# siliconsorcery/crdt

Hardware: AMD Instinct MI355X
Metric: merged records/sec (node) + % HBM roofline, 1B records x 1024 replicas (higher is better)
Workload: dtype int64

## Files before the change

crdt_amd/csrc/crdt_merge.hip:

```cpp
#include <dlfcn.h>
#include <hip/hip_runtime.h>
#include <rccl/rccl.h>

#include <stdint.h>
#include <stdio.h>
#include <stdlib.h>
#include <string.h>

#include <unistd.h>

#include <algorithm>
#include <atomic>
#include <chrono>
#include <thread>
#include <new>
#include <vector>

#include "crdt_merge.h"

namespace {

constexpr int kShift = 16;
constexpr int64_t kMaxCounter = 0xFFFF;
constexpr int64_t kMaxDrift = 60000;
// ... 1752 lines not shown
    uint32_t form_off = 0;
    bool env_dynamic = false;
    bool hist_fuse = true;
    uint32_t l1_tile = 0;
    uint32_t plan_l1_tile = 28672;
    bool last_hist1_fused = false;
    bool frame_lt_only = false;
    const uint32_t* d_ptb = nullptr;
    uint64_t plan_ptiles = 0;
    DBuf<uint32_t> p_hist1;
    bool hist1_fused = false;
    bool hist1_routed = false;
    const uint32_t* hist1_key = nullptr;
    uint32_t hist1_shift = 0;
    bool last_packed = false;
    bool last_wire_pk = false;
    bool last_own_in_place = false;
    bool last_key8 = false;
    bool last_key16 = false;
    bool last_compact = false;
    bool last_hw = false;
    bool flags_sorted = true;
    int fback_chk = 6;
    bool last_flagged = false;
    int combine = 1;
    bool last_combined = false;
    uint32_t sparse_t = 2048;
    uint32_t hot_buckets = 256;
    uint32_t hot_share = 5;
    uint32_t hot_probe = kHotProbe;
    uint32_t hot_skip = 0;
    uint32_t hist1_hot = 0;
    bool last_hot_direct = false;
    DBuf<uint32_t> p_hist1h, p_toffh, p_dstarth;
    DBuf<uint64_t> p_l1begh;
    int route_l1 = 1;
    bool rl1_call_head = false;
    bool rl1_call_all = false;
    bool rl1_cmp = false;
    bool last_rl1_head = false;
    uint64_t last_rl1_head_in = 0, last_rl1_head_out = 0;
    uint32_t last_rl1_head_digits = 0;
    uint64_t sent_bytes = 0;
    uint32_t rl1_pieces = 2;
    uint32_t rl1_call_pieces = 2;
    uint32_t last_rl1_pieces = 0;
    bool last_route_l1 = false;
    bool route_tune = true;
    struct RouteTune {
        uint64_t shape = 0;
        uint32_t trial = 0;
        int best = -1;
        long long us[5] = {-1, -1, -1, -1, -1};
    } rt;
    int tune_mode = -1;
    bool tune_trial = false;
    DBuf<long long> d_tune;
    HBuf<long long> h_tune;
    DBuf<uint32_t> rl_rec;
    DBuf<uint16_t> rl_k16;
    uint64_t rl_cap = 0;
    Rl1Scratch rl_os[kRl1MaxPieces + 1];
    Rl1Scratch rl_hf;
    DBuf<uint32_t> rl_hrec;
    DBuf<uint16_t> rl_hk16;
    DBuf<unsigned long long> rl_hcnt;
// ... 630 lines not shown
                 crdt_result* out, uint8_t* dflags = nullptr,
                 EmitOut* emit = nullptr) {
    const uint32_t R = c->plan_R;
    const bool fl = dflags != nullptr;
    const bool em = emit != nullptr;
    if (!em) {
        if (!c->resolved)
            k_resolve<<<1, 64, 0, c->stream>>>(d_event, R, wall, c->canonical, c->d_Rj.p, c->d_Cj.p, c->d_misc);
        c->resolved = false;
        ev_record(c, kEvApply);
        c->windows.clear();
        c->apply_total = 1;
        if (c->timing) ev_record(c, ev_window(0, false));
    }
    const bool two = c->cap > (1ull << 20);
    const uint32_t shift1 = two ? 20u : (uint32_t)kSBits;
    const size_t ns_all = sg.j.size();
    PackFrame pf{};
    bool pk = false;
    if (cols.packed_in || (c->packed_resolve && c->frame_on)) {
        HIPCHK(hipMemcpyAsync(c->h_misc, c->d_misc, sizeof(Misc), hipMemcpyDeviceToHost, c->stream));
        SYNCHK(c, c->stream);
        pf = frame_of(c);
        pk = pf.ok;
        if (cols.packed_in && !pk) return CRDT_E_INVALID;
    }
    if ((fl || em) && (!pk || cols.packed_in)) return CRDT_E_INVALID;
    const bool ord = !em && (fl || (c->counts && pk && !cols.packed_in));
    c->last_ordered = ord;
    c->last_packed = pk;
    c->key_end_valid = true;
    c->last_hist1_fused = false;
    c->last_hot_direct = false;
    c->sorted_phases = false;
    const bool k8 = pk && two && pf.key4 && !(c->form_off & kFormNoKey8);
    const bool k16 = k8 && !(c->form_off & kFormNoKey16);
    bool cmp = false;
    if (k16 && (ord || !c->counts) && !em && !c->has_comm && !cols.packed_in && c->frame_on &&
        !(c->form_off & (kFormNoCompact | kFormNoHistW | kFormBigTile2 | kFormNoWholeLines | kFormNoVecLoads))) {
        const PackFrame cf = compact_frame(pf, (uint32_t)std::min<unsigned long long>(c->h_misc->fr_cmax, 0xFFFFull),
                                           c->plan_R);
        if (cf.cb) {
            pf = cf;
            cmp = true;
        }
    }
    c->last_compact = cmp;
    c->last_key8 = k8;
    c->last_key16 = k16;
    c->last_hw = pk && (!c->counts || ord) && c->hw_read < c->cap;
    const uint32_t win0 = pk ? pf.jwin : kWindow;
    const bool pt1 = fl && cmp && ns_all && sg.j[0] / win0 == sg.j[ns_all - 1] / win0 &&
                     !(c->form_off & (kFormNoPosT | kFormNoFbackPre | kFormFbackWide)) &&
                     !(c->xcd_map && (c->form_off & kFormFbackXcd));
    if (fl && !pt1) {
        uint64_t ncol = 0;
        for (size_t s = 0; s < ns_all; ++s) ncol = std::max<uint64_t>(ncol, sg.end[s]);
        HIPALLOC(c->f_pos1.ensure((ncol ? ncol : 1) + 8));
    }
    for (size_t sb = 0; sb < ns_all;) {
        const uint32_t win = pk ? pf.jwin : kWindow;
        const uint32_t jb = sg.j[sb] - sg.j[sb] % win;
        size_t se = sb;
        uint64_t nw = 0;
        while (se < ns_all && sg.j[se] < jb + win) { nw += sg.end[se] - sg.beg[se]; ++se; }
        const uint32_t nseg = (uint32_t)(se - sb);
// ... 55 lines not shown
            }
            for (hipEvent_t& e : c->place_ev)
                if (!e) HIPCHK(hipEventCreate(&e));
            c->place_timed = true;
        }
        HIPALLOC(c->p1_rec.ensure(rec_units)); HIPALLOC(c->p1_kj.ensure(kj1_units));
        u32x4* p1r = c->p1_rec.p;
        uint32_t* p1k = c->p1_kj.p;
        u32x4* p2r = nullptr;
        uint32_t* p2k = nullptr;
        const uint64_t* d_beg = c->p_plan.p;
        const uint64_t* d_end = c->p_plan.p + nseg;
        const uint32_t* d_sj = reinterpret_cast<const uint32_t*>(c->p_plan.p + 2 * (size_t)nseg);
        const uint32_t* d_tb1 = d_sj + nseg;
        HIPALLOC(c->p_tseg.ensure(ntm));
        k_seg_index<<<std::min<uint32_t>(grid_for(nt1, 256), 4096), 256, 0, c->stream>>>(d_tb1, nseg, nt1, c->p_tseg.p);
        const TileMap tm1{d_beg, d_end, d_tb1, c->p_tseg.p, d_sj, nseg, l1t};
        const ScanMap sm1z{reinterpret_cast<const uint32_t*>(c->p_plan.p + tail),
                          reinterpret_cast<const uint32_t*>(c->p_plan.p + tail + 1), c->p_plan.p + tail + 2, 1};
        if (two) HIPALLOC(c->p_l1beg.ensure(kDigits + 1));
        const bool h1 = c->hist1_fused && !c->hist1_routed && s0 == 0 && se == ns_all && !cols.packed_in &&
                        cols.key == c->hist1_key && c->hist1_shift == shift1 && nt1 == c->plan_ptiles &&
                        l1t == l1_plan_tile(c);
        const uint32_t* hist1 = h1 ? c->p_hist1.p : c->p_hist.p;
        const uint32_t hb = h1 ? c->hist1_hot : 0u;
        const uint64_t hot_n = hb && pk ? std::min<uint64_t>(c->h_misc->hot_n, nw) : 0;
        const bool hotp = hb && cmp && !ord && !em && two && !c->has_comm && hot_n * 100 >= (uint64_t)c->hot_share * nw;
        if (hb && !hotp) {
            k_hot_fold<<<std::min<uint32_t>(nt1, 1024u), 64, 0, c->stream>>>(c->p_hist1.p, c->p_hist1h.p, nt1);
            c->hist1_hot = 0;
            c->hot_skip = c->hot_probe;
        }
        c->last_hot_direct = hotp;
        if (hotp) {
            HIPALLOC(c->p_toffh.ensure((size_t)nt1 * kDigits));
            HIPALLOC(c->p_dstarth.ensure(kDigits + 1));
            HIPALLOC(c->p_l1begh.ensure(kDigits + 1));
            HIPALLOC(c->p2_rec.ensure(rec_units));
            k_hist_trim<<<256, 256, 0, c->stream>>>(c->p_hist1h.p, c->d_ptb, R, c->d_misc);
            k_scan_part<<<nc1, 256, 0, c->stream>>>(c->p_hist1h.p, sm1z, c->p_part.p);
            k_scan_seg<<<1, 256, 0, c->stream>>>(c->p_part.p, sm1z, c->p_choff.p, c->p_dstarth.p, c->p_l1begh.p);
            k_scan_tiles<<<nc1, 256, 0, c->stream>>>(c->p_hist1h.p, c->p_choff.p, sm1z, c->p_dstarth.p, c->p_toffh.p);
        }
        const ScanMap sm1 = hotp ? ScanMap{sm1z.tbase, sm1z.cbase, c->p_l1begh.p + kDigits, 1} : sm1z;
        if (h1)
            k_hist_trim<<<256, 256, 0, c->stream>>>(c->p_hist1.p, c->d_ptb, R, c->d_misc);
        else
            k_part_hist<true><<<nt1, kHThreads, 0, c->stream>>>(cols.key, tm1, jb, c->d_misc,
                                                                 c->cap, shift1, c->p_hist.p);
        c->last_hist1_fused = h1;
        k_scan_part<<<nc1, 256, 0, c->stream>>>(hist1, sm1, c->p_part.p);
        k_scan_seg<<<1, 256, 0, c->stream>>>(c->p_part.p, sm1, c->p_choff.p, c->p_dstart1.p,
                                             two ? c->p_l1beg.p : nullptr);
        k_scan_tiles<<<nc1, 256, 0, c->stream>>>(hist1, c->p_choff.p, sm1, c->p_dstart1.p, c->p_toff.p);
        const bool ph = c->timing && s0 == 0 && !em;
        if (ph) ev_record(c, ev_window(1, false));
        if (c->place_timed && s0 == 0) HIPCHK(hipEventRecord(c->place_ev[0], c->stream));
        const uint32_t xper1 = c->xcd_map ? (nt1 + kXcds - 1) / kXcds : 0;
        const bool rev1 = c->xcd_map && !(c->form_off & kFormNoReverse);
        if (pt1) HIPALLOC(c->f_pos1.ensure((size_t)nt1 * kPTile + 16));
        if (pt1)
            k_part_scatter1<true, false, true, kL1Items, true, true, true, true, true>
                <<<xcd_grid(nt1, c->xcd_map), kPThreads, 0, c->stream>>>(
                cols.key, cols.lt, cols.rank, cols.val, tm1, jb, c->d_misc, c->cap, shift1, c->p_toff.p, p1r,
                p1k, xper1, pf, rev1 ? hist1 : nullptr, c->f_pos1.p, hist1);
        else if (cmp && fl)
            k_part_scatter1<true, false, true, kL1Items, true, true, true, true>
                <<<xcd_grid(nt1, c->xcd_map), kPThreads, 0, c->stream>>>(
                cols.key, cols.lt, cols.rank, cols.val, tm1, jb, c->d_misc, c->cap, shift1, c->p_toff.p, p1r,
                p1k, xper1, pf, rev1 ? hist1 : nullptr, c->f_pos1.p, hist1);
        else if (hotp)
            k_part_scatter1<kL1Items><<<xcd_grid(nt1, c->xcd_map), kPThreads, 0, c->stream>>>(
                cols.key, cols.lt, cols.rank, cols.val, tm1, jb, c->d_misc, c->cap, shift1, c->p_toff.p, p1r,
                p1k, xper1, pf, rev1 ? hist1 : nullptr,
                HotL1{hb, c->p_toffh.p, rev1 ? c->p_hist1h.p : nullptr, c->p2_rec.p});
        else if (cmp)
            k_part_scatter1<true, false, true, kL1Items, true, true, false, true>
                <<<xcd_grid(nt1, c->xcd_map), kPThreads, 0, c->stream>>>(
                cols.key, cols.lt, cols.rank, cols.val, tm1, jb, c->d_misc, c->cap, shift1, c->p_toff.p, p1r,
                p1k, xper1, pf, rev1 ? hist1 : nullptr);
        else if (fl && k16)
            k_part_scatter1<true, false, true, kL1Items, true, true, true>
                <<<xcd_grid(nt1, c->xcd_map), kPThreads, 0, c->stream>>>(
                cols.key, cols.lt, cols.rank, cols.val, tm1, jb, c->d_misc, c->cap, shift1, c->p_toff.p, p1r,
                p1k, xper1, pf, rev1 ? hist1 : nullptr, c->f_pos1.p, hist1);
        else if (fl)
            k_part_scatter1<true, false, false, kL1Items, true, false, true>
                <<<xcd_grid(nt1, c->xcd_map), kPThreads, 0, c->stream>>>(
                cols.key, cols.lt, cols.rank, cols.val, tm1, jb, c->d_misc, c->cap, shift1, c->p_toff.p, p1r,
                p1k, xper1, pf, rev1 ? hist1 : nullptr, c->f_pos1.p, hist1);
        else if (cols.packed_in && k16)
            k_part_scatter1<true, true, true, kL1Items, true><<<xcd_grid(nt1, c->xcd_map), kPThreads, 0, c->stream>>>(
                cols.key, cols.lt, cols.rank, cols.val, tm1, jb, c->d_misc, c->cap, shift1, c->p_toff.p, p1r,
                p1k, xper1, pf, rev1 ? hist1 : nullptr);
        else if (cols.packed_in)
            k_part_scatter1<true, true, false, kL1Items, true><<<xcd_grid(nt1, c->xcd_map), kPThreads, 0, c->stream>>>(
                cols.key, cols.lt, cols.rank, cols.val, tm1, jb, c->d_misc, c->cap, shift1, c->p_toff.p, p1r,
                p1k, xper1, pf, rev1 ? hist1 : nullptr);
        else if (k16 && !(c->form_off & kFormNoVecLoads))
            k_part_scatter1<true, false, true, kL1Items, true><<<xcd_grid(nt1, c->xcd_map), kPThreads, 0, c->stream>>>(
                cols.key, cols.lt, cols.rank, cols.val, tm1, jb, c->d_misc, c->cap, shift1, c->p_toff.p, p1r,
                p1k, xper1, pf, rev1 ? hist1 : nullptr);
        else if (k16)
// ... 511 lines not shown
        case CRDT_E_NOMEM: return "device out of memory";
        case CRDT_E_KEY_RANGE: return "key id out of range";
        case CRDT_E_NO_DEVICE: return "no gfx950 device";
        case CRDT_E_COMM: return "communicator error";
        default: return "unknown status";
    }
}

int crdt_device_count(int* out) {
    if (!out) return CRDT_E_INVALID;
    int n = 0;
    if (hipGetDeviceCount(&n) != hipSuccess) n = 0;
    *out = n;
    return CRDT_OK;
}

static void read_env_knobs(crdt_ctx* c) {
    if (const char* e = getenv("CRDT_NO_FUSE")) c->no_fuse = atoi(e) != 0;
    if (const char* e = getenv("CRDT_XCD_MAP")) c->xcd_map = atoi(e) != 0;
    if (const char* e = getenv("CRDT_PACKED")) c->packed_resolve = atoi(e) != 0;
    if (const char* e = getenv("CRDT_FLAGS_SORTED")) c->flags_sorted = atoi(e) != 0;
    if (const char* e = getenv("CRDT_TABLE_MERGE")) c->table_merge = atoi(e) != 0;
    if (const char* e = getenv("CRDT_COMBINE")) c->combine = std::min(std::max(atoi(e), 0), 2);
    if (const char* e = getenv("CRDT_ROUTE_L1")) c->route_l1 = std::min(std::max(atoi(e), 0), 3);
    if (const char* e = getenv("CRDT_RL1_SPLIT")) {
        const int v = atoi(e);
        c->rl1_pieces = std::min<uint32_t>(v <= 0 ? 1u : v == 1 ? 2u : (uint32_t)v, kRl1MaxPieces);
    }
    if (const char* e = getenv("CRDT_ROUTE_TUNE")) c->route_tune = atoi(e) != 0;
    if (const char* e = getenv("CRDT_SPARSE_T")) c->sparse_t = (uint32_t)std::max(atoi(e), 0);
    if (const char* e = getenv("CRDT_HOT_BUCKETS")) c->hot_buckets = (uint32_t)std::min(std::max(atoi(e), 0), (int)kHotMax);
    if (const char* e = getenv("CRDT_HOT_PROBE")) c->hot_probe = (uint32_t)std::min(std::max(atoi(e), 0), 1 << 20);
    if (const char* e = getenv("CRDT_HOT_SHARE")) c->hot_share = (uint32_t)std::min(std::max(atoi(e), 0), 100);
    if (const char* e = getenv("CRDT_FBACK_CHK")) c->fback_chk = atoi(e) == 4 ? 4 : atoi(e) == 0 ? 0 : 6;
    if (const char* e = getenv("CRDT_HIST_FUSE")) c->hist_fuse = atoi(e) != 0;
    if (const char* e = getenv("CRDT_L1_TILE"))
        c->l1_tile = std::min<uint32_t>((uint32_t)std::max(atoi(e), 0) / 1024u * 1024u, (uint32_t)kPTile);
    if (const char* e = getenv("CRDT_SORTED_FORM")) c->form_off = (uint32_t)strtoul(e, nullptr, 10);
    if (const char* e = getenv("CRDT_APPLY_ITEMS")) {
        const int v = atoi(e);
        c->apply_items = (v == 1 || v == 2 || v == 4 || v == 8) ? v : 0;
    }
    c->fail_rank = -1;
    c->fail_at = 0;
    if (const char* e = getenv("CRDT_TEST_FAIL")) {
        int r = -1, at = 0;
        if (sscanf(e, "%d:%d", &r, &at) == 2) { c->fail_rank = r; c->fail_at = at; }
    }
    c->stall_rank = -1;
    c->stall_at = c->stall_ms = 0;
    c->stall_dev = false;
    if (const char* e = getenv("CRDT_TEST_STALL")) {
        int r = -1, at = 0, ms = 0;
        char d = 0;
        const int k = sscanf(e, "%d:%d:%d:%c", &r, &at, &ms, &d);
        if (k >= 3) { c->stall_rank = r; c->stall_at = at; c->stall_ms = ms; c->stall_dev = k == 4 && d == 'd'; }
    }
}

int crdt_create(int device, uint32_t local_rank, uint64_t capacity, crdt_ctx** out) {
    if (!out) return CRDT_E_INVALID;
    *out = nullptr;
    int n = 0;
    if (hipGetDeviceCount(&n) != hipSuccess || device < 0 || device >= n) return CRDT_E_NO_DEVICE;
    hipDeviceProp_t prop;
    if (hipGetDeviceProperties(&prop, device) != hipSuccess) return CRDT_E_NO_DEVICE;
// ... 1252 lines not shown
int crdt_set_merge_path(crdt_ctx* c, int path) {
    if (!c || path < CRDT_PATH_AUTO || path > CRDT_PATH_SORTED) return CRDT_E_INVALID;
    c->merge_path = path;
    return CRDT_OK;
}

int crdt_last_path(const crdt_ctx* c, int* path) {
    if (!c || !path) return CRDT_E_INVALID;
    *path = c->last_sorted ? CRDT_PATH_SORTED : CRDT_PATH_GATHER;
    return CRDT_OK;
}

int crdt_last_plan(const crdt_ctx* c, uint32_t* flags) {
    if (!c || !flags) return CRDT_E_INVALID;
    uint32_t f = 0;
    if (c->last_table_plan) {
        *flags = c->last_table_plan;
        return CRDT_OK;
    }
    if (c->last_sorted) {
        f |= CRDT_PLAN_SORTED;
        if (c->last_packed) f |= CRDT_PLAN_PACKED;
        if (c->cap > (1ull << 20)) f |= CRDT_PLAN_TWO_LEVEL;
        if (c->last_hist1_fused) f |= CRDT_PLAN_HIST_IN_SCAN;
        if (c->last_key8) f |= CRDT_PLAN_KEY8;
        if (c->last_key16) f |= CRDT_PLAN_KEY16;
        if (c->last_hw) f |= CRDT_PLAN_HIGH_WATER;
        if (c->last_flagged) f |= CRDT_PLAN_FLAGGED;
        if (c->last_ordered) f |= CRDT_PLAN_ORDERED;
        if (c->last_combined) f |= CRDT_PLAN_COMBINED;
        if (c->last_route_l1) f |= CRDT_PLAN_ROUTE_L1;
        if (c->last_compact) f |= CRDT_PLAN_COMPACT;
        if (c->last_hot_direct) f |= CRDT_PLAN_HOT_DIRECT;
    }
    if (c->last_wire_pk) f |= CRDT_PLAN_WIRE_PACKED;
    if (c->last_own_in_place) f |= CRDT_PLAN_OWN_IN_PLACE;
    if (c->tune_trial) f |= CRDT_PLAN_ROUTE_TUNED;
    if (c->last_route_l1) f |= (c->last_rl1_pieces & 7u) << CRDT_PLAN_RL1_PIECES_SHIFT;
    if (c->last_route_l1 && c->last_rl1_head) f |= CRDT_PLAN_RL1_HEAD;
    *flags = f;
    return CRDT_OK;
}

int crdt_place_info(const crdt_ctx* c, int32_t* n, int32_t* kept, int32_t* done, float* ms) {
    if (!c || !n || !kept || !done || !ms) return CRDT_E_INVALID;
    *n = c->place_k;
    *kept = c->place_best;
    *done = c->place_k > 1 ? c->place_trial + 1 : 0;
    for (int i = 0; i < crdt_ctx::kPlaceMax; ++i) ms[i] = i < c->place_k ? c->place_ms[i] : 0.f;
    return CRDT_OK;
}

int crdt_route_tune_info(const crdt_ctx* c, int32_t* best, int64_t* us) {
    if (!c || !best || !us) return CRDT_E_INVALID;
    *best = c->rt.best;
    for (int w = 0; w < 5; ++w) us[w] = c->rt.us[w];
    return CRDT_OK;
}

int crdt_set_timing(crdt_ctx* c, int enable) {
    if (!c) return CRDT_E_INVALID;
    c->timing = enable != 0;
    return CRDT_OK;
}

int crdt_get_timing(const crdt_ctx* c, crdt_timing* out) {
// ... 7 lines not shown
```

crdt_amd/csrc/sorted_path.inc:

```

constexpr int kSBits = 12;
constexpr uint32_t kSKeys = 1u << kSBits;
constexpr uint32_t kDigits = 256;
constexpr int kJShift = 20;
constexpr uint32_t kKeyLoMask = (1u << kJShift) - 1;
constexpr uint32_t kWindow = 1u << (32 - kJShift);
constexpr int kHThreads = 1024;
constexpr int kPThreads = 1024;
constexpr int kPWaves = kPThreads / 64;
constexpr int kPItems = 4;
constexpr int kPSub = kPThreads * kPItems;
constexpr int kPTile = 28672;
constexpr int kPTile2 = 8192;
constexpr int kPGroups = kPItems * kPWaves;
#ifndef CRDT_FREE_ITEMS
#define CRDT_FREE_ITEMS 7
#endif
#ifndef CRDT_L1_ITEMS
#define CRDT_L1_ITEMS 7
#endif
constexpr int kFreeItems = CRDT_FREE_ITEMS;
constexpr int kL1Items = CRDT_L1_ITEMS;
constexpr int kPLanes = kPThreads / 256;
static_assert(kPGroups / kPLanes == 16, "group scan: 16 groups per lane");
// ... 694 lines not shown
        for (int q = 0; q < kI; ++q) {
            const uint32_t s2 = q * kPThreads + tid;
            if (s2 >= n) continue;
            Rec12 o;
            o.a = s_pay[0][s2];
            o.b = s_pay[1][s2];
            o.c = s_pay[2][s2];
            const uint32_t kj = kC ? o.b : s_kj[kC ? 0 : s2];
            const uint32_t dd = (kj >> shift) & (kDigits - 1);
            const uint64_t g = (uint64_t)cur[dd] + (s2 - cnt[dd]);
            if (kK8 && !kIn16 && !kC) o.b |= (kj & 15u) << 28;
            orec[g] = o;
            if (kC) {
            } else if (kK8) {
                static_cast<uint8_t*>(okj)[g] = (uint8_t)(kIn16 ? kj : kj >> 4);
            } else {
                static_cast<uint32_t*>(okj)[g] = kj;
            }
        }
        __syncthreads();
        if (tid < (int)kDigits) cur[tid] += (tid + 1 < (int)kDigits ? cnt[tid + 1] : n) - cnt[tid];
        sb += n;
        __syncthreads();
    }
}

struct HotL1 {
    uint32_t hot = 0;
    const uint32_t* toff = nullptr;
    const uint32_t* thist = nullptr;
    void* orec = nullptr;
};

__device__ inline uint32_t scan512_excl(uint32_t v, uint32_t* s_w , uint32_t* total) {
    const int tid = threadIdx.x, lane = tid & 63, w = tid >> 6;
    uint32_t inc = v;
#pragma unroll
    for (int off = 1; off < 64; off <<= 1) {
        const uint32_t u = __shfl_up(inc, off, 64);
        if (lane >= off) inc += u;
    }
    if (tid < 512 && lane == 63) s_w[w] = inc;
    __syncthreads();
    uint32_t x = lane < 8 ? s_w[lane] : 0u;
#pragma unroll
    for (int off = 1; off < 8; off <<= 1) {
        const uint32_t u = __shfl_up(x, off, 64);
        if (lane >= off) x += u;
    }
    const int wu = __builtin_amdgcn_readfirstlane(w);
    *total = (uint32_t)__builtin_amdgcn_readlane((int)x, 7);
    const uint32_t wp = wu == 0 ? 0u : wu <= 8 ? (uint32_t)__builtin_amdgcn_readlane((int)x, wu - 1) : *total;
    return wp + inc - v;
}

__device__ inline uint32_t digit_count_s(uint32_t* bins, uint32_t d, bool act) {
    const unsigned long long a = __ballot(act);
    if (!a) return 0;
    const int L = __ffsll((long long)a) - 1;
    const uint32_t d0 = (uint32_t)__builtin_amdgcn_readlane((int)d, L);
    const bool same = act && d == d0;
    const unsigned long long m = __ballot(same);
    const uint32_t below = __builtin_amdgcn_mbcnt_hi((uint32_t)(m >> 32), __builtin_amdgcn_mbcnt_lo((uint32_t)m, 0u));
    uint32_t base = 0;
    if (same && below == 0) base = atomicAdd(&bins[d0], (uint32_t)__popcll(m));
    base = (uint32_t)__builtin_amdgcn_readlane((int)base, L);
    if (same) return base + below;
    return act ? atomicAdd(&bins[d], 1u) : 0u;
}

template <bool kPk, bool kPkIn, bool kK16, int kItems, bool kVec, bool kDigKj, bool kPos, bool kC, bool kPT, bool kHot>
__device__ __forceinline__ void part_scatter1_body(
    const uint32_t* __restrict__ keyw, const int64_t* __restrict__ lt, const uint32_t* __restrict__ rank,
    const uint32_t* __restrict__ val, TileMap tm, uint32_t jbase, Misc* __restrict__ misc, uint64_t cap,
    uint32_t shift, const uint32_t* __restrict__ toff, void* __restrict__ orec, void* __restrict__ okj,
    uint32_t xper, PackFrame pf, const uint32_t* __restrict__ thist,
    uint16_t* __restrict__ pos_out, const uint32_t* __restrict__ phist, KeyMap km, HotL1 hl)
{
    static_assert(!kK16 || kPk, "2-B key column: packed records only");
    static_assert(!kDigKj || kK16, "digit beside the 16-bit key: 2-B key columns only");
    static_assert(!kC || (kK16 && kDigKj && !kPkIn), "compact: one ctx's packed forms");
    static_assert(!kPT || (kPos && kVec && (kPThreads * kItems) % 8 == 0), "tile-strided positions: kVec groups");
    static_assert(!kHot || (kC && !kPos && kPThreads >= 512), "hot buckets: the compact order-free form");
    constexpr int kW = kPk ? 3 : 4;
    constexpr int kI = kItems;
    constexpr int kS = kPThreads * kI;
    constexpr int kND = kHot ? 2 * (int)kDigits : (int)kDigits;
    __shared__ uint32_t cur[kND];
    __shared__ uint32_t cnt[kND];
    __shared__ uint32_t dst[kND + 1];
    __shared__ uint32_t s_w[kHot ? 8 : 4];
    __shared__ u32x4 s_rec[kPk ? 1 : kS];
    __shared__ uint32_t s_pay[kPk ? kW : 1][kPk ? kS : 1];
    __shared__ uint32_t s_kj[kS];
    __shared__ uint8_t s_dig[kDigKj ? 1 : kS];
    __shared__ uint32_t s_t0[kPos ? kDigits : 1];
    __shared__ uint16_t s_pos[kPos && !kPT ? kS : 1];
    const uint32_t t = tm.tile0 + xcd_tile(blockIdx.x, xper, xper != 0);
    if (t >= tm.tbase[tm.nseg]) return;
    uint32_t seg, len;
    uint64_t beg;
    tile_info(tm, t, &seg, &beg, &len);
    const uint32_t jw = tm.seg_j[seg];
    if (jw >= misc->stop) return;
    const int tid = threadIdx.x, lane = tid & 63;
    const bool rev = thist && (t & 1u);
    if (tid < (int)kDigits)
        cur[tid] = toff[(uint64_t)t * kDigits + tid] + (rev ? thist[(uint64_t)t * kDigits + tid] : 0u);
    else if (kHot && tid < kND)
        cur[tid] = hl.toff[(uint64_t)t * kDigits + tid - kDigits] +
                   (rev ? hl.thist[(uint64_t)t * kDigits + tid - kDigits] : 0u);
    if constexpr (kPos) {
        uint32_t all;
        const uint32_t hv = tid < (int)kDigits ? phist[(uint64_t)t * kDigits + tid] : 0u;
        const uint32_t ex = scan256_excl(hv, s_w, &all);
        if (tid < (int)kDigits) s_t0[kPos ? tid : 0] = ex - toff[(uint64_t)t * kDigits + tid];
    }
    bool bad = false, over = false;
    int64_t nl[kI];
    uint32_t nr[kI], nvl[kI], nk[kI];
    static_assert(!kVec || kI >= 4, "kVec: 4 consecutive records per thread");
    constexpr int kG4 = kVec ? kI / 4 : 0, kP2 = kVec && kI % 4 >= 2 ? 1 : 0;
    auto rec_index = [&](uint32_t sb, int q) -> uint32_t {
        if (q < 4 * kG4) return sb + (uint32_t)(q >> 2) * (4u * kPThreads) + (uint32_t)tid * 4u + (uint32_t)(q & 3);
        const uint32_t b2 = sb + 4u * kG4 * kPThreads;
        if (kP2 && q < 4 * kG4 + 2) return b2 + (uint32_t)tid * 2u + (uint32_t)(q - 4 * kG4);
        return kVec ? b2 + 2u * kP2 * kPThreads + (uint32_t)(q - 4 * kG4 - 2 * kP2) * kPThreads + tid
                    : sb + (uint32_t)q * kPThreads + tid;
    };
    auto load1 = [&](uint32_t sb, int q) {
        const uint32_t i = rec_index(sb, q);
        const uint64_t gi = beg + (i < len ? i : 0);
        nl[q] = __builtin_nontemporal_load(lt + gi);
        nr[q] = kPkIn ? 0u : __builtin_nontemporal_load(rank + gi);
        nvl[q] = __builtin_nontemporal_load(val + gi);
        nk[q] = __builtin_nontemporal_load(keyw + gi);
    };
    auto load_sub = [&](uint32_t sb) {
#pragma unroll
        for (int g4 = 0; g4 < kG4; ++g4) {
            const int q = 4 * g4;
            const uint32_t i0 = rec_index(sb, q);
            if (i0 + 4u <= len) {
                const uint64_t g = beg + i0;
// ... 12 lines not shown
                    nr[q] = nr[q + 1] = nr[q + 2] = nr[q + 3] = 0u;
                }
            } else {
#pragma unroll
                for (int j = 0; j < 4; ++j) load1(sb, q + j);
            }
        }
        if constexpr (kP2 != 0) {
            const int q = 4 * kG4;
            const uint32_t i0 = rec_index(sb, q);
            if (i0 + 2u <= len) {
                const uint64_t g = beg + i0;
                const u32x2u kv = *reinterpret_cast<const u32x2u*>(keyw + g);
                const u32x2u vv = *reinterpret_cast<const u32x2u*>(val + g);
                const u32x4u l0 = *reinterpret_cast<const u32x4u*>(lt + g);
                nk[q] = kv.x; nk[q + 1] = kv.y;
                nvl[q] = vv.x; nvl[q + 1] = vv.y;
                nl[q] = (int64_t)(((uint64_t)l0.y << 32) | l0.x); nl[q + 1] = (int64_t)(((uint64_t)l0.w << 32) | l0.z);
                if constexpr (!kPkIn) {
                    const u32x2u rv = *reinterpret_cast<const u32x2u*>(rank + g);
                    nr[q] = rv.x; nr[q + 1] = rv.y;
                } else {
                    nr[q] = nr[q + 1] = 0u;
                }
            } else {
                load1(sb, q);
                load1(sb, q + 1);
            }
        }
#pragma unroll
        for (int q = 4 * kG4 + 2 * kP2; q < kI; ++q) load1(sb, q);
    };
    load_sub(0);
    for (uint32_t sb = 0; sb < len; sb += kS) {
        if (tid < kND) cnt[tid] = 0;
        uint32_t rec[kI][kW];
        uint32_t k[kI], d[kI], slot[kI];
        bool act[kI];
#pragma unroll
        for (int q = 0; q < kI; ++q) {
            act[q] = rec_index(sb, q) < len;
            if (kPk && !kPkIn) over |= act[q] && nr[q] >= pf.rk_limit;
            if constexpr (kPk) {
                int64_t lq = nl[q];
                uint64_t pk;
                pk = kPkIn ? (uint64_t)nl[q] : pack_record<kC>(pf, lq, nr[q], jw - jbase);
                rec[q][0] = (uint32_t)pk;
                rec[q][1] = (uint32_t)(pk >> 32);
                rec[q][kW - 1] = nvl[q];
            } else {
                rec[q][0] = (uint32_t)nl[q];
                rec[q][1] = (uint32_t)((uint64_t)nl[q] >> 32);
                rec[q][2] = nr[q];
                rec[q][kW - 1] = nvl[q];
            }
            k[q] = nk[q];
        }
        if (sb + kS < len) load_sub(sb + kS);
        __syncthreads();
#pragma unroll
        for (int q = 0; q < kI; ++q) {
            const uint32_t sl = k[q] >> km.gsh;
            bad |= act[q] && sl >= cap;
            act[q] = act[q] && sl < cap;
            d[q] = km_digit(km, k[q], shift);
            if (kHot) d[q] = (sl >> kSBits) < hl.hot ? kDigits + (sl >> kSBits) : d[q];
            if (kC) {
                rec[q][1] |= (sl & 0xFFFFFu) << (kCKeyShift - 32);
                k[q] = (sl >> 12) & 0xFFu;
                if (kHot) k[q] |= d[q] << 16;
            } else if (kK16) {
                rec[q][1] |= (sl & 15u) << 28;
                k[q] = (sl >> 4) & 0xFFFFu;
            } else {
                k[q] = (sl & kKeyLoMask) | ((jw - jbase) << kJShift);
            }
            slot[q] = kHot ? digit_count_s(cnt, d[q], act[q]) : digit_count(cnt, d[q], act[q], lane);
        }
        __syncthreads();
        uint32_t all;
        const uint32_t tv = tid < kND ? cnt[tid] : 0u;
        const uint32_t ex = kHot ? scan512_excl(tv, s_w, &all) : scan256_excl(tv, s_w, &all);
        if (tid < kND) {
            dst[tid] = ex;
            if (tid == kND - 1) dst[kND] = ex + tv;
            if (rev) cur[tid] -= tv;
        }
        __syncthreads();
#pragma unroll
        for (int q = 0; q < kI; ++q) {
            if (act[q]) {
                const uint32_t pos = dst[kHot ? k[q] >> 16 : d[q]] + slot[q];
                if constexpr (kPk) {
#pragma unroll
                    for (int x = 0; x < kW; ++x) s_pay[x][pos] = rec[q][x];
                } else {
                    u32x4 r4; r4.x = rec[q][0]; r4.y = rec[q][1]; r4.z = rec[q][2]; r4.w = rec[q][kW - 1];
                    s_rec[pos] = r4;
                }
                if (kHot) {
                    s_kj[pos] = k[q];
                } else if (kDigKj) {
                    s_kj[pos] = k[q] | (d[q] << 16);
                } else {
                    s_kj[pos] = k[q];
                    s_dig[kDigKj ? 0 : pos] = (uint8_t)d[q];
                }
                if constexpr (kPos && !kPT)
                    s_pos[kPos && !kPT ? rec_index(sb, q) - sb : 0] =
                        (uint16_t)(cur[d[q]] + slot[q] + s_t0[kPos ? d[q] : 0]);
            }
        }
        if constexpr (kPT) {
            uint32_t pp[kI];
#pragma unroll
            for (int q = 0; q < kI; ++q) pp[q] = act[q] ? (cur[d[q]] + slot[q] + s_t0[kPos ? d[q] : 0]) & 0xFFFFu : 0u;
            uint16_t* __restrict__ po = pos_out + (uint64_t)t * kPTile;
#pragma unroll
            for (int g4 = 0; g4 < kG4; ++g4) {
                const int q = 4 * g4;
                const uint32_t i0 = rec_index(sb, q);
                if (i0 + 4u <= len) {
                    u32x2u v;
                    v.x = pp[q] | (pp[q + 1] << 16);
                    v.y = pp[q + 2] | (pp[q + 3] << 16);
                    *reinterpret_cast<u32x2u*>(po + i0) = v;
                } else {
#pragma unroll
                    for (int u = 0; u < 4; ++u)
                        if (i0 + u < len) po[i0 + u] = (uint16_t)pp[q + u];
                }
            }
            if constexpr (kP2 != 0) {
                const int q = 4 * kG4;
                const uint32_t i0 = rec_index(sb, q);
                if (i0 + 2u <= len) *reinterpret_cast<uint32_t*>(po + i0) = pp[q] | (pp[q + 1] << 16);
                else if (i0 < len) po[i0] = (uint16_t)pp[q];
            }
#pragma unroll
            for (int q = 4 * kG4 + 2 * kP2; q < kI; ++q) {
                const uint32_t i = rec_index(sb, q);
                if (i < len) po[i] = (uint16_t)pp[q];
            }
        }
        __syncthreads();
        const uint32_t staged = dst[kND];
        if constexpr (kPos && !kPT) {
            const uint32_t ns = std::min<uint32_t>((uint32_t)kS, len - sb);
            uint16_t* __restrict__ po = pos_out + beg + sb;
            const uint32_t head = std::min<uint32_t>(ns, (8u - (uint32_t)(((uintptr_t)po >> 1) & 7u)) & 7u);
            const uint32_t nv = (ns - head) / 8u;
            if ((uint32_t)tid < head) po[tid] = s_pos[kPos ? tid : 0];
            for (uint32_t i = tid; i < nv; i += kPThreads) {
                const uint32_t b = head + i * 8u;
                u32x4 v;
                v.x = (uint32_t)s_pos[kPos ? b : 0] | ((uint32_t)s_pos[kPos ? b + 1 : 0] << 16);
                v.y = (uint32_t)s_pos[kPos ? b + 2 : 0] | ((uint32_t)s_pos[kPos ? b + 3 : 0] << 16);
                v.z = (uint32_t)s_pos[kPos ? b + 4 : 0] | ((uint32_t)s_pos[kPos ? b + 5 : 0] << 16);
                v.w = (uint32_t)s_pos[kPos ? b + 6 : 0] | ((uint32_t)s_pos[kPos ? b + 7 : 0] << 16);
                *reinterpret_cast<u32x4*>(po + b) = v;
            }
            const uint32_t tl = head + nv * 8u;
            if (tl + (uint32_t)tid < ns) po[tl + tid] = s_pos[kPos ? tl + tid : 0];
        }
#pragma unroll
        for (int q = 0; q < kI; ++q) {
            const uint32_t s = q * kPThreads + tid;
            if (s < staged) {
                const uint32_t kw = s_kj[s];
                const uint32_t dd = kDigKj ? kw >> 16 : s_dig[kDigKj ? 0 : s];
                const uint64_t g = (uint64_t)cur[dd] + (s - dst[dd]);
                if constexpr (kPk) {
                    uint32_t o[kW];
#pragma unroll
                    for (int x = 0; x < kW; ++x) o[x] = s_pay[x][s];
                    store_payload<kPk>(kHot && dd >= kDigits ? hl.orec : orec, g, o);
                } else {
                    static_cast<u32x4*>(orec)[g] = s_rec[s];
                }
                if (kHot && dd >= kDigits) continue;
                if (kC) static_cast<uint8_t*>(okj)[g] = (uint8_t)kw;
                else if (kK16) static_cast<uint16_t*>(okj)[g] = (uint16_t)kw;
                else static_cast<uint32_t*>(okj)[g] = kw;
            }
        }
        __syncthreads();
        if (tid < kND && !rev) cur[tid] += dst[tid + 1] - dst[tid];
    }
    const unsigned long long em = kHot ? __ballot(true) : 0ull;
    const bool l0 = kHot ? __builtin_amdgcn_mbcnt_hi((uint32_t)(em >> 32), __builtin_amdgcn_mbcnt_lo((uint32_t)em, 0u)) == 0u
                         : lane == 0;
    if (__any(bad) && l0) atomicOr(&misc->err, 1u);
    if (kPk && __any(over) && l0) atomicOr(&misc->err, 2u);
}

template <bool kPk, bool kPkIn = false, bool kK16 = false, int kItems = kL1Items, bool kVec = false,
          bool kDigKj = kK16, bool kPos = false, bool kC = false, bool kPT = false>
__global__ __launch_bounds__(kPThreads) void k_part_scatter1(
    const uint32_t* __restrict__ keyw, const int64_t* __restrict__ lt, const uint32_t* __restrict__ rank,
    const uint32_t* __restrict__ val, TileMap tm, uint32_t jbase, Misc* __restrict__ misc, uint64_t cap,
    uint32_t shift, const uint32_t* __restrict__ toff, void* __restrict__ orec, void* __restrict__ okj,
    uint32_t xper, PackFrame pf, const uint32_t* __restrict__ thist,
    uint16_t* __restrict__ pos_out = nullptr, const uint32_t* __restrict__ phist = nullptr,
    KeyMap km = KeyMap{0u, 8u})
{
    part_scatter1_body<kPk, kPkIn, kK16, kItems, kVec, kDigKj, kPos, kC, kPT, false>(
        keyw, lt, rank, val, tm, jbase, misc, cap, shift, toff, orec, okj, xper, pf, thist, pos_out, phist, km, HotL1{});
}

template <int kItems = kL1Items>
__global__ __launch_bounds__(kPThreads) void k_part_scatter1(
    const uint32_t* __restrict__ keyw, const int64_t* __restrict__ lt, const uint32_t* __restrict__ rank,
    const uint32_t* __restrict__ val, TileMap tm, uint32_t jbase, Misc* __restrict__ misc, uint64_t cap,
    uint32_t shift, const uint32_t* __restrict__ toff, void* __restrict__ orec, void* __restrict__ okj,
    uint32_t xper, PackFrame pf, const uint32_t* __restrict__ thist, HotL1 hl)
{
    part_scatter1_body<true, false, true, kItems, true, true, false, true, false, true>(
        keyw, lt, rank, val, tm, jbase, misc, cap, shift, toff, orec, okj, xper, pf, thist, nullptr, nullptr,
        KeyMap{0u, 8u}, hl);
}

constexpr uint32_t kRPart = 32 * kRChunk;
constexpr uint32_t kJLocal = 0xFFFFFFFFu;
constexpr uint32_t kJAbsent = 0xFFFFFFFEu;

struct KeyState {
    int64_t* lt;
    uint32_t* rank;
    uint32_t* val;
    uint32_t* j;
};

__device__ inline uint32_t bucket_parts(const uint32_t* bstart, uint32_t b) {
    const uint32_t n = bstart[b + 1] - bstart[b];
    return (n + kRPart - 1) / kRPart;
}

__global__ __launch_bounds__(1024) void k_bucket_items(const uint32_t* __restrict__ bstart, uint32_t nb,
                                                       uint32_t* __restrict__ ibase, uint32_t* __restrict__ hbase,
                                                       uint32_t* __restrict__ hot, Misc* __restrict__ misc,
                                                       uint32_t* __restrict__ ebase = nullptr)
{
    __shared__ uint32_t s_p[16], s_hp[16], s_cp[16], s_w[16], s_h[16], s_c[16], s_e[16], s_ep[16], s_ew[16];
    const uint32_t tid = threadIdx.x, lane = tid & 63, w = tid >> 6;
    const uint32_t b0 = blockIdx.x * 1024u;
    auto parts = [&](uint32_t k) { return (bstart[k + 1] - bstart[k] + kRPart - 1) / kRPart; };
    auto eslots = [&](uint32_t k) { return std::min<uint32_t>(kSKeys, bstart[k + 1] - bstart[k]); };
    uint32_t pre = 0, hpre = 0, cpre = 0, epre = 0;
#pragma unroll 8
    for (uint32_t k = tid; k < b0; k += 1024) {
// ... 1307 lines not shown
```

crdt_amd/device.py:

```python
from __future__ import annotations

import ctypes

import numpy as np

from . import _capi
from ._capi import CrdtBatch, CrdtResult, CrdtTiming


class CrdtNativeError(RuntimeError):
    def __init__(self, status: int, what: str = ""):
        self.status = status
        msg = _capi.status_string(status) if status else "ok"
        super().__init__(f"{what}: {msg} ({status})" if what else f"{msg} ({status})")


def _is_torch(a) -> bool:
    return type(a).__module__.startswith("torch")


_NP_TYPES = {"u4": np.uint32, "i8": np.int64, "u1": np.uint8}
_TORCH_KINDS = {"u4": ("int32", "uint32"), "i8": ("int64",), "u1": ("uint8", "bool")}


# ... 448 lines not shown
    def comm_free(self):
        self._check(self._lib.crdt_comm_free(self._ctx), "crdt_comm_free")

    def set_presharded(self, on: bool):
        self._check(self._lib.crdt_set_presharded(self._ctx, 1 if on else 0), "crdt_set_presharded")

    PATHS = {"auto": 0, "gather": 1, "sorted": 2}

    def set_counts(self, exact: bool):
        self._check(self._lib.crdt_set_counts(self._ctx, 1 if exact else 0), "crdt_set_counts")

    def set_row_bytes(self, row_bytes: int):
        self._check(self._lib.crdt_set_row_bytes(self._ctx, int(row_bytes)), "crdt_set_row_bytes")

    def reserve_scratch(self, n_records: int):
        self._check(self._lib.crdt_reserve_scratch(self._ctx, int(n_records)), "crdt_reserve_scratch")

    def set_rank_bound(self, bound: int):
        self._check(self._lib.crdt_set_rank_bound(self._ctx, int(bound)), "crdt_set_rank_bound")

    def set_merge_path(self, path: str):
        self._check(self._lib.crdt_set_merge_path(self._ctx, self.PATHS[path]), "crdt_set_merge_path")

    def last_path(self) -> str:
        v = ctypes.c_int(0)
        self._check(self._lib.crdt_last_path(self._ctx, ctypes.byref(v)), "crdt_last_path")
        return {1: "gather", 2: "sorted"}[v.value]

    PLAN_FLAGS = {"sorted": 1, "packed": 2, "two_level": 4, "hist_in_scan": 8, "key8": 16, "key16": 32,
                  "high_water": 64, "anchored": 128, "wire_packed": 256, "own_in_place": 512,
                  "flagged": 1024, "ordered": 2048,
                  "combined": 4096, "route_l1": 8192, "route_tuned": 16384, "rl1_head": 262144,
                  "compact": 524288, "hot_direct": 1048576, "table": 2097152,
                  "sync": 4194304, "fanin": 8388608, "fanout": 16777216}

    def last_plan(self) -> dict:
        v = ctypes.c_uint32(0)
        self._check(self._lib.crdt_last_plan(self._ctx, ctypes.byref(v)), "crdt_last_plan")
        plan = {k: bool(v.value & b) for k, b in self.PLAN_FLAGS.items()}
        plan["rl1_pieces"] = (v.value >> 15) & 7
        return plan

    def place_info(self) -> dict:
        n, kept, done = ctypes.c_int32(0), ctypes.c_int32(0), ctypes.c_int32(0)
        ms = (ctypes.c_float * 4)()
        self._check(self._lib.crdt_place_info(self._ctx, ctypes.byref(n), ctypes.byref(kept), ctypes.byref(done), ms),
                    "crdt_place_info")
        return {"candidates": n.value, "kept": kept.value if kept.value >= 0 else None, "merges_used": done.value,
                "level1_ms": [round(float(m), 3) for m in ms[:max(n.value, 0)]]}

    TUNE_WAYS = ("route_l1", "combine", "route_l1_4", "route_l1_1", "route_l1_head")

    def route_tune(self) -> dict:
        best = ctypes.c_int32(0)
        us = (ctypes.c_int64 * 5)()
        self._check(self._lib.crdt_route_tune_info(self._ctx, ctypes.byref(best), us), "crdt_route_tune_info")
        out = {"best": self.TUNE_WAYS[best.value] if 0 <= best.value < len(self.TUNE_WAYS) else None}
        for w, u in zip(self.TUNE_WAYS, us):
            out[f"{w}_ms"] = u / 1e3 if u >= 0 else None
        return out

    def set_timing(self, enable: bool):
        self._check(self._lib.crdt_set_timing(self._ctx, int(bool(enable))), "crdt_set_timing")

    def timing(self) -> dict:
        t = CrdtTiming()
        self._check(self._lib.crdt_get_timing(self._ctx, ctypes.byref(t)), "crdt_get_timing")
# ... 2 lines not shown
```

include/crdt_merge.h:

```cpp
#ifndef CRDT_MERGE_H
#define CRDT_MERGE_H

#include <stdint.h>

#ifdef __cplusplus
extern "C" {
#endif

#define CRDT_ABI_VERSION 5
#define CRDT_NULL_VALUE 0xFFFFFFFFu

enum crdt_status {
    CRDT_OK = 0,
    CRDT_CLOCK_DRIFT = 1,
    CRDT_DUPLICATE_NODE = 2,
    CRDT_OVERFLOW = 3,
    CRDT_E_INVALID = -1,
    CRDT_E_HIP = -2,
    CRDT_E_NOMEM = -3,
    CRDT_E_KEY_RANGE = -4,
    CRDT_E_NO_DEVICE = -5,
    CRDT_E_COMM = -6
};

// ... 165 lines not shown
int crdt_set_comm_timeout(crdt_ctx* ctx, uint32_t ms);
int crdt_comm_state(const crdt_ctx* ctx, int32_t* state, const char** phase);
int crdt_set_presharded(crdt_ctx* ctx, int presharded);

enum crdt_path { CRDT_PATH_AUTO = 0, CRDT_PATH_GATHER = 1, CRDT_PATH_SORTED = 2 };
int crdt_set_merge_path(crdt_ctx* ctx, int path);

int crdt_set_counts(crdt_ctx* ctx, int exact);
int crdt_set_rank_bound(crdt_ctx* ctx, uint32_t bound);
int crdt_last_path(const crdt_ctx* ctx, int* path);
enum crdt_plan_flags {
    CRDT_PLAN_SORTED = 1,
    CRDT_PLAN_PACKED = 2,
    CRDT_PLAN_TWO_LEVEL = 4,
    CRDT_PLAN_HIST_IN_SCAN = 8,
    CRDT_PLAN_KEY8 = 16,
    CRDT_PLAN_KEY16 = 32,
    CRDT_PLAN_HIGH_WATER = 64,
    CRDT_PLAN_ANCHORED = 128,
    CRDT_PLAN_WIRE_PACKED = 256,
    CRDT_PLAN_OWN_IN_PLACE = 512,
    CRDT_PLAN_FLAGGED = 1024,
    CRDT_PLAN_ORDERED = 2048,
    CRDT_PLAN_COMBINED = 4096,
    CRDT_PLAN_ROUTE_L1 = 8192,
    CRDT_PLAN_ROUTE_TUNED = 16384,
    CRDT_PLAN_RL1_PIECES_SHIFT = 15,
    CRDT_PLAN_RL1_HEAD = 262144,
    CRDT_PLAN_COMPACT = 524288,
    CRDT_PLAN_HOT_DIRECT = 1048576,
    CRDT_PLAN_TABLE = 2097152,
    CRDT_PLAN_SYNC = 4194304,
    CRDT_PLAN_FANIN = 8388608,
    CRDT_PLAN_FANOUT = 16777216
};
int crdt_last_plan(const crdt_ctx* ctx, uint32_t* flags);

int crdt_route_tune_info(const crdt_ctx* ctx, int32_t* best, int64_t* us );

int crdt_place_info(const crdt_ctx* ctx, int32_t* n, int32_t* kept, int32_t* done, float* ms );

int crdt_set_timing(crdt_ctx* ctx, int enable);
int crdt_get_timing(const crdt_ctx* ctx, crdt_timing* out);

#ifdef __cplusplus
}
#endif
#endif
```

Baseline: 56.10 billion.

## Carry partial-line run tails across sub-tiles in hot-bucket L1 scatter

Adds a run-tail carry mode to the hot-bucket level-1 scatter kernel. Each digit's records that would land in a partially written 64-byte line at the end of a sub-tile are held in shared memory and written together with the next sub-tile's records, so global writes cover whole lines. The aim is to reduce partial-line writes and the HBM read-modify-write traffic they cause. The cost is extra shared memory, per-digit bookkeeping, two-thread-per-digit carry loops and more index arithmetic. It is on by default and can be turned off with an environment variable.

```diff
diff --git a/crdt_amd/csrc/crdt_merge.hip b/crdt_amd/csrc/crdt_merge.hip
--- a/crdt_amd/csrc/crdt_merge.hip
+++ b/crdt_amd/csrc/crdt_merge.hip
@@ -1808,6 +1808,8 @@
     uint32_t hot_skip = 0;
     uint32_t hist1_hot = 0;
     bool last_hot_direct = false;
+    bool l1_carry = true;
+    bool last_l1_carry = false;
     DBuf<uint32_t> p_hist1h, p_toffh, p_dstarth;
     DBuf<uint64_t> p_l1begh;
     int route_l1 = 1;
@@ -2504,6 +2506,7 @@
     c->key_end_valid = true;
     c->last_hist1_fused = false;
     c->last_hot_direct = false;
+    c->last_l1_carry = false;
     c->sorted_phases = false;
     const bool k8 = pk && two && pf.key4 && !(c->form_off & kFormNoKey8);
     const bool k16 = k8 && !(c->form_off & kFormNoKey16);
@@ -2625,6 +2628,7 @@
             c->hot_skip = c->hot_probe;
         }
         c->last_hot_direct = hotp;
+        c->last_l1_carry = hotp && c->l1_carry;
         if (hotp) {
             HIPALLOC(c->p_toffh.ensure((size_t)nt1 * kDigits));
             HIPALLOC(c->p_dstarth.ensure(kDigits + 1));
@@ -2662,6 +2666,11 @@
                 <<<xcd_grid(nt1, c->xcd_map), kPThreads, 0, c->stream>>>(
                 cols.key, cols.lt, cols.rank, cols.val, tm1, jb, c->d_misc, c->cap, shift1, c->p_toff.p, p1r,
                 p1k, xper1, pf, rev1 ? hist1 : nullptr, c->f_pos1.p, hist1);
+        else if (hotp && c->l1_carry)
+            k_part_scatter1<kL1Items, true><<<xcd_grid(nt1, c->xcd_map), kPThreads, 0, c->stream>>>(
+                cols.key, cols.lt, cols.rank, cols.val, tm1, jb, c->d_misc, c->cap, shift1, c->p_toff.p, p1r,
+                p1k, xper1, pf, rev1 ? hist1 : nullptr,
+                HotL1{hb, c->p_toffh.p, rev1 ? c->p_hist1h.p : nullptr, c->p2_rec.p});
         else if (hotp)
             k_part_scatter1<kL1Items><<<xcd_grid(nt1, c->xcd_map), kPThreads, 0, c->stream>>>(
                 cols.key, cols.lt, cols.rank, cols.val, tm1, jb, c->d_misc, c->cap, shift1, c->p_toff.p, p1r,
@@ -3239,6 +3248,7 @@
     if (const char* e = getenv("CRDT_HOT_BUCKETS")) c->hot_buckets = (uint32_t)std::min(std::max(atoi(e), 0), (int)kHotMax);
     if (const char* e = getenv("CRDT_HOT_PROBE")) c->hot_probe = (uint32_t)std::min(std::max(atoi(e), 0), 1 << 20);
     if (const char* e = getenv("CRDT_HOT_SHARE")) c->hot_share = (uint32_t)std::min(std::max(atoi(e), 0), 100);
+    if (const char* e = getenv("CRDT_L1_CARRY")) c->l1_carry = atoi(e) != 0;
     if (const char* e = getenv("CRDT_FBACK_CHK")) c->fback_chk = atoi(e) == 4 ? 4 : atoi(e) == 0 ? 0 : 6;
     if (const char* e = getenv("CRDT_HIST_FUSE")) c->hist_fuse = atoi(e) != 0;
     if (const char* e = getenv("CRDT_L1_TILE"))
@@ -4557,6 +4567,7 @@
         if (c->last_route_l1) f |= CRDT_PLAN_ROUTE_L1;
         if (c->last_compact) f |= CRDT_PLAN_COMPACT;
         if (c->last_hot_direct) f |= CRDT_PLAN_HOT_DIRECT;
+        if (c->last_l1_carry) f |= CRDT_PLAN_L1_CARRY;
     }
     if (c->last_wire_pk) f |= CRDT_PLAN_WIRE_PACKED;
     if (c->last_own_in_place) f |= CRDT_PLAN_OWN_IN_PLACE;
diff --git a/crdt_amd/csrc/sorted_path.inc b/crdt_amd/csrc/sorted_path.inc
--- a/crdt_amd/csrc/sorted_path.inc
+++ b/crdt_amd/csrc/sorted_path.inc
@@ -750,6 +750,9 @@
     void* orec = nullptr;
 };
 
+constexpr uint32_t kL1Gran = 64;
+constexpr uint32_t l1_carry_recs(uint32_t g_words) { return (g_words + 3u) / 3u; }
+
 __device__ inline uint32_t scan512_excl(uint32_t v, uint32_t* s_w , uint32_t* total) {
     const int tid = threadIdx.x, lane = tid & 63, w = tid >> 6;
     uint32_t inc = v;
@@ -787,7 +790,8 @@
     return act ? atomicAdd(&bins[d], 1u) : 0u;
 }
 
-template <bool kPk, bool kPkIn, bool kK16, int kItems, bool kVec, bool kDigKj, bool kPos, bool kC, bool kPT, bool kHot>
+template <bool kPk, bool kPkIn, bool kK16, int kItems, bool kVec, bool kDigKj, bool kPos, bool kC, bool kPT, bool kHot,
+          bool kCarry>
 __device__ __forceinline__ void part_scatter1_body(
     const uint32_t* __restrict__ keyw, const int64_t* __restrict__ lt, const uint32_t* __restrict__ rank,
     const uint32_t* __restrict__ val, TileMap tm, uint32_t jbase, Misc* __restrict__ misc, uint64_t cap,
@@ -800,6 +804,7 @@
     static_assert(!kC || (kK16 && kDigKj && !kPkIn), "compact: one ctx's packed forms");
     static_assert(!kPT || (kPos && kVec && (kPThreads * kItems) % 8 == 0), "tile-strided positions: kVec groups");
     static_assert(!kHot || (kC && !kPos && kPThreads >= 512), "hot buckets: the compact order-free form");
+    static_assert(!kCarry || kHot, "run-tail carry: the hot-bucket form");
     constexpr int kW = kPk ? 3 : 4;
     constexpr int kI = kItems;
     constexpr int kS = kPThreads * kI;
@@ -810,8 +815,15 @@
     __shared__ uint32_t s_w[kHot ? 8 : 4];
     __shared__ u32x4 s_rec[kPk ? 1 : kS];
     __shared__ uint32_t s_pay[kPk ? kW : 1][kPk ? kS : 1];
-    __shared__ uint32_t s_kj[kS];
+    __shared__ uint32_t s_kj[kCarry ? 1 : kS];
     __shared__ uint8_t s_dig[kDigKj ? 1 : kS];
+    constexpr uint32_t kG = kL1Gran / 4u;
+    constexpr int kCR = kCarry ? (int)l1_carry_recs(kG) : 1;
+    __shared__ uint16_t s_d16[kCarry ? kS : 1];
+    __shared__ uint32_t s_carry[kCarry ? kW : 1][kCarry ? kCR * kND : 1];
+    static_assert(!kCarry || kPThreads == 2 * kND, "run-tail carry: two threads per digit");
+    __shared__ uint32_t s_ncar[2][kCarry ? kND : 1];
+    __shared__ uint32_t s_lim[kCarry ? kND : 1];
     __shared__ uint32_t s_t0[kPos ? kDigits : 1];
     __shared__ uint16_t s_pos[kPos && !kPT ? kS : 1];
     const uint32_t t = tm.tile0 + xcd_tile(blockIdx.x, xper, xper != 0);
@@ -828,6 +840,9 @@
     else if (kHot && tid < kND)
         cur[tid] = hl.toff[(uint64_t)t * kDigits + tid - kDigits] +
                    (rev ? hl.thist[(uint64_t)t * kDigits + tid - kDigits] : 0u);
+    if constexpr (kCarry) {
+        if (tid < kND) s_ncar[0][tid] = 0;
+    }
     if constexpr (kPos) {
         uint32_t all;
         const uint32_t hv = tid < (int)kDigits ? phist[(uint64_t)t * kDigits + tid] : 0u;
@@ -906,6 +921,7 @@
         for (int q = 4 * kG4 + 2 * kP2; q < kI; ++q) load1(sb, q);
     };
     load_sub(0);
+    uint32_t cp = 0;
     for (uint32_t sb = 0; sb < len; sb += kS) {
         if (tid < kND) cnt[tid] = 0;
         uint32_t rec[kI][kW];
@@ -959,6 +975,19 @@
             dst[tid] = ex;
             if (tid == kND - 1) dst[kND] = ex + tv;
             if (rev) cur[tid] -= tv;
+            if constexpr (kCarry) {
+                uint32_t tq = (uint32_t)tid;
+                asm volatile("" : "+v"(tq));
+                const uint32_t st = s_ncar[cp][kCarry ? tq : 0], nc = st & 0xFFu, part = st >> 8;
+                const uint32_t base = (uint32_t)(reinterpret_cast<uintptr_t>(tq >= kDigits ? hl.orec : orec) >> 2);
+                const uint32_t far = rev ? cur[tid] : cur[tid] + tv;
+                const uint32_t e = (base + 3u * far) & (kG - 1u);
+                const uint32_t past = sb + kS >= len ? 0u : rev ? (kG - e) & (kG - 1u) : e;
+                const uint32_t endv = 3u * (nc + tv);
+                const uint32_t hiv = endv - std::min(past, endv - part);
+                const uint32_t w = hiv >= 3u * nc ? (hiv - 3u * nc) / 3u : 0u;
+                s_lim[kCarry ? tq : 0] = (rev ? ex + tv - w : ex + w) | (hiv << 16);
+            }
         }
         __syncthreads();
 #pragma unroll
@@ -972,7 +1001,9 @@
                     u32x4 r4; r4.x = rec[q][0]; r4.y = rec[q][1]; r4.z = rec[q][2]; r4.w = rec[q][kW - 1];
                     s_rec[pos] = r4;
                 }
-                if (kHot) {
+                if constexpr (kCarry) {
+                    s_d16[pos] = (uint16_t)(k[q] >> 16);
+                } else if (kHot) {
                     s_kj[pos] = k[q];
                 } else if (kDigKj) {
                     s_kj[pos] = k[q] | (d[q] << 16);
@@ -1037,11 +1068,73 @@
             const uint32_t tl = head + nv * 8u;
             if (tl + (uint32_t)tid < ns) po[tl + tid] = s_pos[kPos ? tl + tid : 0];
         }
-#pragma unroll
-        for (int q = 0; q < kI; ++q) {
+        if constexpr (kCarry) {
+            auto store_words = [&](void* __restrict__ ob, uint64_t g, const uint32_t (&o)[kW], uint32_t lo, uint32_t hi) {
+                if (lo == 0u && hi >= 3u) {
+                    store_payload<kPk>(ob, g, o);
+                    return;
+                }
+                uint32_t* __restrict__ p = static_cast<uint32_t*>(ob) + 3u * g;
+#pragma unroll
+                for (int x = 0; x < 3; ++x)
+                    if ((uint32_t)x >= lo && (uint32_t)x < hi) p[rev ? 2 - x : x] = o[rev ? 2 - x : x];
+            };
+            uint32_t tl = (uint32_t)tid;
+            asm volatile("" : "+v"(tl));
+#pragma unroll
+            for (int q = 0; q < kI; ++q) {
+                const uint32_t s = q * kPThreads + tl;
+                if (s < staged) {
+                    const uint32_t dd = s_d16[kCarry ? s : 0];
+                    const uint32_t thr = s_lim[kCarry ? dd : 0] & 0xFFFFu;
+                    const uint64_t g = (uint64_t)cur[dd] + (s - dst[dd]);
+                    uint32_t o[kW];
+#pragma unroll
+                    for (int x = 0; x < kW; ++x) o[x] = s_pay[x][s];
+                    if (rev ? s >= thr : s < thr) store_payload<kPk>(dd >= kDigits ? hl.orec : orec, g, o);
+                    if (dd < kDigits) static_cast<uint8_t*>(okj)[g] = (uint8_t)(o[1] >> 24);
+                }
+            }
+            {
+                const uint32_t dg = tl & (uint32_t)(kND - 1), par = tl / (uint32_t)kND;
+                const uint32_t st = s_ncar[cp][kCarry ? dg : 0], nc = st & 0xFFu, part = st >> 8;
+                const uint32_t n = dst[dg + 1] - dst[dg];
+                const uint32_t hiv = s_lim[kCarry ? dg : 0] >> 16;
+                void* const ob = dg >= kDigits ? hl.orec : orec;
+                const uint64_t g0 = rev ? (uint64_t)cur[dg] + n + nc - 1u : (uint64_t)cur[dg] - nc;
+                if (hiv >= 3u * nc) {
+#pragma nounroll
+                    for (uint32_t r = par; r < (uint32_t)kCR; r += 2u) {
+                        if (r < nc) {
+                            uint32_t o[kW];
+#pragma unroll
+                            for (int x = 0; x < kW; ++x) o[x] = s_carry[x][kCarry ? r * kND + dg : 0];
+                            store_words(ob, rev ? g0 - r : g0 + r, o, r == 0u ? part : 0u, 3u);
+                        }
+                    }
+                }
+                const uint32_t first = hiv / 3u, ncn = nc + n - first, partn = hiv - 3u * first;
+#pragma nounroll
+                for (uint32_t r2 = par; r2 < (uint32_t)kCR; r2 += 2u) {
+                    const uint32_t r = first + r2;
+                    if (r2 < ncn && r >= nc) {
+                        const uint32_t sj = rev ? dst[dg + 1] - 1u - (r - nc) : dst[dg] + (r - nc);
+                        uint32_t o[kW];
+#pragma unroll
+                        for (int x = 0; x < kW; ++x) o[x] = s_pay[x][sj];
+#pragma unroll
+                        for (int x = 0; x < kW; ++x) s_carry[x][kCarry ? r2 * kND + dg : 0] = o[x];
+                        if (r2 == 0u && partn) store_words(ob, rev ? g0 - r : g0 + r, o, 0u, partn);
+                    }
+                }
+                if (par == 0u) s_ncar[cp ^ 1u][kCarry ? dg : 0] = ncn | (partn << 8);
+            }
+        }
+#pragma unroll
+        for (int q = 0; q < (kCarry ? 0 : kI); ++q) {
             const uint32_t s = q * kPThreads + tid;
             if (s < staged) {
-                const uint32_t kw = s_kj[s];
+                const uint32_t kw = s_kj[kCarry ? 0 : s];
                 const uint32_t dd = kDigKj ? kw >> 16 : s_dig[kDigKj ? 0 : s];
                 const uint64_t g = (uint64_t)cur[dd] + (s - dst[dd]);
                 if constexpr (kPk) {
@@ -1060,6 +1153,7 @@
         }
         __syncthreads();
         if (tid < kND && !rev) cur[tid] += dst[tid + 1] - dst[tid];
+        if constexpr (kCarry) cp ^= 1u;
     }
     const unsigned long long em = kHot ? __ballot(true) : 0ull;
     const bool l0 = kHot ? __builtin_amdgcn_mbcnt_hi((uint32_t)(em >> 32), __builtin_amdgcn_mbcnt_lo((uint32_t)em, 0u)) == 0u
@@ -1078,18 +1172,18 @@
     uint16_t* __restrict__ pos_out = nullptr, const uint32_t* __restrict__ phist = nullptr,
     KeyMap km = KeyMap{0u, 8u})
 {
-    part_scatter1_body<kPk, kPkIn, kK16, kItems, kVec, kDigKj, kPos, kC, kPT, false>(
+    part_scatter1_body<kPk, kPkIn, kK16, kItems, kVec, kDigKj, kPos, kC, kPT, false, false>(
         keyw, lt, rank, val, tm, jbase, misc, cap, shift, toff, orec, okj, xper, pf, thist, pos_out, phist, km, HotL1{});
 }
 
-template <int kItems = kL1Items>
+template <int kItems = kL1Items, bool kCarry = false>
 __global__ __launch_bounds__(kPThreads) void k_part_scatter1(
     const uint32_t* __restrict__ keyw, const int64_t* __restrict__ lt, const uint32_t* __restrict__ rank,
     const uint32_t* __restrict__ val, TileMap tm, uint32_t jbase, Misc* __restrict__ misc, uint64_t cap,
     uint32_t shift, const uint32_t* __restrict__ toff, void* __restrict__ orec, void* __restrict__ okj,
     uint32_t xper, PackFrame pf, const uint32_t* __restrict__ thist, HotL1 hl)
 {
-    part_scatter1_body<true, false, true, kItems, true, true, false, true, false, true>(
+    part_scatter1_body<true, false, true, kItems, true, true, false, true, false, true, kCarry>(
         keyw, lt, rank, val, tm, jbase, misc, cap, shift, toff, orec, okj, xper, pf, thist, nullptr, nullptr,
         KeyMap{0u, 8u}, hl);
 }
diff --git a/crdt_amd/device.py b/crdt_amd/device.py
--- a/crdt_amd/device.py
+++ b/crdt_amd/device.py
@@ -504,7 +504,7 @@
                   "flagged": 1024, "ordered": 2048,
                   "combined": 4096, "route_l1": 8192, "route_tuned": 16384, "rl1_head": 262144,
                   "compact": 524288, "hot_direct": 1048576, "table": 2097152,
-                  "sync": 4194304, "fanin": 8388608, "fanout": 16777216}
+                  "sync": 4194304, "fanin": 8388608, "fanout": 16777216, "l1_carry": 33554432}
 
     def last_plan(self) -> dict:
         v = ctypes.c_uint32(0)
diff --git a/include/crdt_merge.h b/include/crdt_merge.h
--- a/include/crdt_merge.h
+++ b/include/crdt_merge.h
@@ -221,7 +221,8 @@
     CRDT_PLAN_TABLE = 2097152,
     CRDT_PLAN_SYNC = 4194304,
     CRDT_PLAN_FANIN = 8388608,
-    CRDT_PLAN_FANOUT = 16777216
+    CRDT_PLAN_FANOUT = 16777216,
+    CRDT_PLAN_L1_CARRY = 33554432
 };
 int crdt_last_plan(const crdt_ctx* ctx, uint32_t* flags);
 
```

After: 51.43 billion. 8.3% lower.
